# Stan994265/mVIL-Fusion

Hardware: AMD Instinct MI355X
Metric: sliding-window solve iterations/sec (10 KF, 1k feat, 30k LiDAR pts) (higher is better)
Workload: dtype f64; 1 GPU; BASELINE.json configs[1]: K=10 keyframes, L=1000 landmarks, 3068 visual factors, 24000 plane + 6000 edge LiDAR points, 9 IMU, 3 ICP, 4 LPS, prior n=70 (vil_marginalize of the preceding synthetic window, on the GPU); termination=function_tolerance, parallelism=1 GPU, step=one full window solve, inputs resident in HBM

## Files before the change

mvil-fusion_amd/csrc/vil_step.hpp:

```cpp
#pragma once
#include <type_traits>

#include "vil_dev.hpp"
#include "vil_factors.hpp"
#include "vil_finish.hpp"

namespace vd {

#define STEP_NB 4
#define CH_SLOTS 7
#define PF_N ((55 * 256 + VIL_STEP_THREADS - 1) / VIL_STEP_THREADS)

struct StepShared {
    Ctl c;
    double red[64];
    unsigned char tI[256], tJ[256];
    double xs[320], dinv[320];
    double y[320];
    double sc[320], dcs[320], gr[320], gn[320];
    double gd[320];
    double rt[320];
    double x0[328];
    unsigned char cst[48];
    double hs[12];
    int need, was_first, ok, cok;
    int hdr_posted, hdr_pad_;
    int early, judged;
    int done_at_entry, pad0_;
    long long tacc[6];
};

template <bool CMAX = false>
__device__ __forceinline__ void bsum3(double& a, double& b, double& c, StepShared& s) {
    a = wave_total_l63(a); b = wave_total_l63(b);
    c = CMAX ? wave_max_l63(c) : wave_total_l63(c);
    __syncthreads();
    const int w = vil_tid() >> 6, nw = blockDim.x >> 6;
    if ((vil_tid() & 63) == 63) { s.red[w] = a; s.red[8 + w] = b; s.red[16 + w] = c; }
    __syncthreads();
    a = 0; b = 0; c = 0;
    for (int q = 0; q < nw; ++q) { a += s.red[q]; b += s.red[8 + q]; c = CMAX ? fmax(c, s.red[16 + q]) : c + s.red[16 + q]; }
}

__device__ __forceinline__ void bsum5(double& a, double& b, double& c, double& d, double& e, StepShared& s) {
    a = wave_total_l63(a); b = wave_total_l63(b); c = wave_max_l63(c); d = wave_total_l63(d); e = wave_total_l63(e);
    __syncthreads();
    const int w = vil_tid() >> 6, nw = blockDim.x >> 6;
    if ((vil_tid() & 63) == 63) { s.red[w] = a; s.red[8 + w] = b; s.red[16 + w] = c; s.red[24 + w] = d; s.red[32 + w] = e; }
    __syncthreads();
    a = 0; b = 0; c = 0; d = 0; e = 0;
    for (int q = 0; q < nw; ++q) { a += s.red[q]; b += s.red[8 + q]; c = fmax(c, s.red[16 + q]); d += s.red[24 + q]; e += s.red[32 + q]; }
}

__device__ __forceinline__ void bsum6(double* v, StepShared& s) {
#pragma unroll
    for (int e = 0; e < 6; ++e) v[e] = wave_total_l63(v[e]);
    __syncthreads();
    const int w = vil_tid() >> 6, nw = blockDim.x >> 6;
    if ((vil_tid() & 63) == 63) { for (int e = 0; e < 6; ++e) s.red[8 * e + w] = v[e]; }
    __syncthreads();
#pragma unroll
    for (int e = 0; e < 6; ++e) { double a = 0; for (int q = 0; q < nw; ++q) a += s.red[8 * e + q]; v[e] = a; }
}

__device__ __forceinline__ double bsum(double v, StepShared& s) {
    v = wave_total_l63(v);
    __syncthreads();
    if ((vil_tid() & 63) == 63) s.red[vil_tid() >> 6] = v;
    __syncthreads();
    double t = 0;
    const int nw = blockDim.x >> 6;
    for (int w = 0; w < nw; ++w) t += s.red[w];
    return t;
}
__device__ __forceinline__ double bmax(double v, StepShared& s) {
    v = wave_max_l63(v);
    __syncthreads();
    if ((vil_tid() & 63) == 63) s.red[vil_tid() >> 6] = v;
    __syncthreads();
    double t = 0;
    const int nw = blockDim.x >> 6;
    for (int w = 0; w < nw; ++w) t = fmax(t, s.red[w]);
    return t;
}

struct LmRows { double e[13], a[6], b[6], c[6]; double m1, m2; int fs, fe, ac, c0, c1, c2, stride = 3; };
template <bool AG = false>
__device__ __forceinline__ void lm_rows(const DevP& P, const SysBuf& sb, int l, LmRows& r) {
    r.fs = P.glm_start[l]; r.fe = P.glm_start[l + 1]; r.ac = P.glm_acol[l];
    if (r.fe == r.fs) return;
    const double* e = sb.eA + (size_t)l * 13;
#pragma unroll
    for (int k = 0; k < 13; ++k) r.e[k] = ldx<AG>(e + k);
    const int f = r.fs, f1 = min(f + 1, r.fe - 1), f2 = min(f + 2, r.fe - 1);
    r.c0 = P.gfcol[f]; r.c1 = P.gfcol[f1]; r.c2 = P.gfcol[f2];
    const double* e0 = sb.eO + (size_t)f * 6; const double* e1 = sb.eO + (size_t)f1 * 6; const double* e2 = sb.eO + (size_t)f2 * 6;
#pragma unroll
    for (int k = 0; k < 6; ++k) { r.a[k] = ldx<AG>(e0 + k); r.b[k] = ldx<AG>(e1 + k); r.c[k] = ldx<AG>(e2 + k); }
    r.m1 = (f + 1 < r.fe) ? 1.0 : 0.0; r.m2 = (f + 2 < r.fe) ? 1.0 : 0.0;
}
template <bool AG = false>
__device__ __forceinline__ void lm_rows_quad(const DevP& P, const SysBuf& sb, int l, int qd, LmRows& r, const int G = 4 ) {
    const int fs0 = P.glm_start[l], fe = P.glm_start[l + 1];
    r.ac = qd == 0 ? P.glm_acol[l] : 0; r.stride = 3 * G;
    r.fs = min(fs0 + 3 * qd, fe); r.fe = fe;
    if (fe == fs0) { r.fs = fe; return; }
    const double* e = sb.eA + (size_t)l * 13;
#pragma unroll
    for (int k = 0; k < 13; ++k) { const double v = ldx<AG>(e + k); r.e[k] = qd == 0 ? v : 0.0; }
    const int f = min(fs0 + 3 * qd, fe - 1), f1 = min(f + 1, fe - 1), f2 = min(f + 2, fe - 1);
    r.c0 = P.gfcol[f]; r.c1 = P.gfcol[f1]; r.c2 = P.gfcol[f2];
    const double* e0 = sb.eO + (size_t)f * 6; const double* e1 = sb.eO + (size_t)f1 * 6; const double* e2 = sb.eO + (size_t)f2 * 6;
    const bool m0 = fs0 + 3 * qd < fe;
#pragma unroll
    for (int k = 0; k < 6; ++k) { const double va = ldx<AG>(e0 + k); r.a[k] = m0 ? va : 0.0; r.b[k] = ldx<AG>(e1 + k); r.c[k] = ldx<AG>(e2 + k); }
    r.m1 = (fs0 + 3 * qd + 1 < fe) ? 1.0 : 0.0; r.m2 = (fs0 + 3 * qd + 2 < fe) ? 1.0 : 0.0;
}
__device__ __forceinline__ double quad_total(double v) { v = dpp_add<0xB1, 0xf>(v); return dpp_add<0x4E, 0xf>(v); }
__device__ __forceinline__ double pair_total(double v) { return dpp_add<0xB1, 0xf>(v); }
template <bool AG = false>
__device__ __forceinline__ double lm_dot_rows(const DevP& P, const SysBuf& sb, const LmRows& r, const double* vc) {
    if (r.fe == r.fs) return 0.0;
    const double* e = r.e;
    const double* va = vc + r.ac; const double* vx = vc + col_ex(P);
    double s0 = e[0] * va[0], s1 = e[1] * va[1], s2 = e[2] * va[2], s3 = e[3] * va[3];
    s0 += e[4] * va[4]; s1 += e[5] * va[5];
    s2 += e[6] * vx[0]; s3 += e[7] * vx[1]; s0 += e[8] * vx[2]; s1 += e[9] * vx[3]; s2 += e[10] * vx[4]; s3 += e[11] * vx[5];
    s0 += e[12] * vc[col_td(P)];
    {
        const double* v0 = vc + r.c0; const double* v1 = vc + r.c1; const double* v2 = vc + r.c2;
        const double* a = r.a; const double* b = r.b; const double* c = r.c;
        s0 += a[0] * v0[0]; s1 += a[1] * v0[1]; s2 += a[2] * v0[2]; s3 += a[3] * v0[3]; s0 += a[4] * v0[4]; s1 += a[5] * v0[5];
        s2 += r.m1 * (b[0] * v1[0] + b[1] * v1[1] + b[2] * v1[2]); s3 += r.m1 * (b[3] * v1[3] + b[4] * v1[4] + b[5] * v1[5]);
        s0 += r.m2 * (c[0] * v2[0] + c[1] * v2[1] + c[2] * v2[2]); s1 += r.m2 * (c[3] * v2[3] + c[4] * v2[4] + c[5] * v2[5]);
    }
    for (int f = r.fs + r.stride; f < r.fe; f += r.stride) {
        const int f1 = min(f + 1, r.fe - 1), f2 = min(f + 2, r.fe - 1);
        const int c0 = P.gfcol[f], c1 = P.gfcol[f1], c2 = P.gfcol[f2];
        const double* e0 = sb.eO + (size_t)f * 6; const double* e1 = sb.eO + (size_t)f1 * 6; const double* e2 = sb.eO + (size_t)f2 * 6;
        double a[6], b[6], c[6];
#pragma unroll
        for (int k = 0; k < 6; ++k) { a[k] = ldx<AG>(e0 + k); b[k] = ldx<AG>(e1 + k); c[k] = ldx<AG>(e2 + k); }
        const double* v0 = vc + c0; const double* v1 = vc + c1; const double* v2 = vc + c2;
        const double m1 = (f + 1 < r.fe) ? 1.0 : 0.0, m2 = (f + 2 < r.fe) ? 1.0 : 0.0;
        s0 += a[0] * v0[0]; s1 += a[1] * v0[1]; s2 += a[2] * v0[2]; s3 += a[3] * v0[3]; s0 += a[4] * v0[4]; s1 += a[5] * v0[5];
        s2 += m1 * (b[0] * v1[0] + b[1] * v1[1] + b[2] * v1[2]); s3 += m1 * (b[3] * v1[3] + b[4] * v1[4] + b[5] * v1[5]);
        s0 += m2 * (c[0] * v2[0] + c[1] * v2[1] + c[2] * v2[2]); s1 += m2 * (c[3] * v2[3] + c[4] * v2[4] + c[5] * v2[5]);
    }
    return (s0 + s1) + (s2 + s3);
}
template <bool AG = false>
__device__ __forceinline__ double lm_dot(const DevP& P, const SysBuf& sb, int l, const double* vc) {
    LmRows r; lm_rows<AG>(P, sb, l, r);
    return lm_dot_rows<AG>(P, sb, r, vc);
}

__device__ __forceinline__ double quad_form(const DevP& P, const SysBuf& sb, const double* vc, const double* vl, StepShared& s) {
    const int D = P.D, L = P.L, t = vil_tid(), NT = blockDim.x;
    double part = 0;
    for (int e = t; e < D * D; e += NT) { const int i = e / D, j = e - i * D; part += vc[i] * sb.S[e] * vc[j]; }
    for (int l = t; l < L; l += NT) {
        const double ip = sb.invp[l];
        if (ip == 0.0) continue;
        const double ev = lm_dot(P, sb, l, vc);
        part += ip * ev * ev + 2.0 * vl[l] * ev + sb.hll[l] * vl[l] * vl[l];
    }
    return bsum(part, s);
}

__device__ __forceinline__ void pose_plus(const double* in, const double* d, double* o) {
    for (int k = 0; k < 3; ++k) o[k] = in[k] + d[k];
    Q4 q = qmul(qload(in + 3), Q4{1.0, 0.5 * d[3], 0.5 * d[4], 0.5 * d[5]});
    const double n = 1.0 / sqrt(q.w * q.w + q.x * q.x + q.y * q.y + q.z * q.z);
    o[3] = q.x * n; o[4] = q.y * n; o[5] = q.z * n; o[6] = q.w * n;
}


__host__ __device__ constexpr int tri_row_c(int q) { int I = 0; while ((I + 1) * (I + 2) / 2 <= q) ++I; return I; }
__host__ __device__ constexpr int tri_col_c(int q) { return q - tri_row_c(q) * (tri_row_c(q) + 1) / 2; }
template <int N, class F> __device__ __forceinline__ void static_for(F&& f) {
    if constexpr (N > 0) { static_for<N - 1>(f); f(std::integral_constant<int, N - 1>{}); }
}
static_assert(VIL_STEP_THREADS == 512, "the tile <-> element mapping above assumes two tiles per 512-thread stride");

__device__ __forceinline__ int tri_off(int i) { return (i * (i + 1)) >> 1; }
}
#include "vil_chain.hpp"
#include "vil_prechain.hpp"
namespace vd {

#define TILE_RS 17
#define TILE_SZ (16 * TILE_RS)
__device__ __forceinline__ int tl_base(int I, int J) { return (tri_off(I) + J) * TILE_SZ; }
__device__ __forceinline__ int tl_idx(int i, int j) { return tl_base(i >> 4, j >> 4) + (i & 15) * TILE_RS + (j & 15); }
__device__ __forceinline__ int tl_phys(int e) { return (e >> 8) * TILE_SZ + ((e >> 4) & 15) * TILE_RS + (e & 15); }

struct NoPre { template <class C> __device__ __forceinline__ void operator()(C*, const int*) const {} };
template <bool REGRES, class PTR, class PRE = NoPre>
__device__ __forceinline__ bool chol_blocked(PTR A, int D, StepShared& s, double* Acol = nullptr, PRE pre = PRE()) {
    const int t = vil_tid(), NT = blockDim.x, wave = t >> 6, lane = t & 63, NW = NT >> 6;
    const int R = D + 1;
    const int T = (R + 15) >> 4;
    const int la = (lane & 15) * TILE_RS + (lane >> 4);
    const int lc = (lane >> 4) * TILE_RS + (lane & 15);
#ifdef VIL_STAMPS
    long long tacc[6] = {0, 0, 0, 0, 0, 0}, tprev = 0;
    #define CSTAMP(k) do { long long tt_; asm volatile("s_memtime %0\n s_waitcnt lgkmcnt(0)" : "=s"(tt_) :: "memory"); if (k >= 0) tacc[k < 0 ? 0 : k] += tt_ - tprev; tprev = tt_; } while (0)
#else
    #define CSTAMP(k) do {} while (0)
#endif
    const int ntile_all = (T * (T + 1)) >> 1;
    d4 Creg[REGRES ? CH_SLOTS : 1]; int tIJ[REGRES ? CH_SLOTS : 1];
    if constexpr (REGRES) {
#pragma unroll
        for (int u = 0; u < CH_SLOTS; ++u) {
            const int g = wave + NW * u;
            tIJ[u] = -1;
            if (g < ntile_all) {
                const int I = s.tI[g], J = s.tJ[g];
                tIJ[u] = (I << 8) | J;
                const int cb = tl_base(I, J) + lc;
#pragma unroll
                for (int q = 0; q < 4; ++q) Creg[u][q] = A[cb + q * (4 * TILE_RS)];
            }
        }
        pre(Creg, tIJ);
    }
    for (int kb = 0; kb < D; kb += STEP_NB) {
        const int nb = min(STEP_NB, D - kb);
        const int Kt = kb >> 4, ko = kb & 15;
        CSTAMP(-1);
        if constexpr (REGRES) if (ko == 0) {
#pragma unroll
            for (int u = 0; u < CH_SLOTS; ++u) if (tIJ[u] >= 0 && (tIJ[u] & 255) == Kt) {
                const int cb = tl_base(tIJ[u] >> 8, Kt) + lc;
#pragma unroll
                for (int q = 0; q < 4; ++q) A[cb + q * (4 * TILE_RS)] = Creg[u][q];
            }
            __syncthreads();
            CSTAMP(4);
        }
        if constexpr (!REGRES) if (ko == 0) {
            __syncthreads();
            for (int e = t; e < (T - Kt) * TILE_SZ; e += NT) { const int I = Kt + e / TILE_SZ, w = e - (I - Kt) * TILE_SZ; Acol[e] = A[tl_base(I, Kt) + w]; }
            __syncthreads();
        }
        double* const AC = REGRES ? (double*)A : Acol;
        auto cbase = [&](int I) { return REGRES ? tl_base(I, Kt) : (I - Kt) * TILE_SZ; };
        const int db = cbase(Kt) + ko * TILE_RS + ko;
        double d00 = AC[db], d10 = 0, d11 = 1, d20 = 0, d21 = 0, d22 = 1, d30 = 0, d31 = 0, d32 = 0, d33 = 1;
        if (nb > 1) { d10 = AC[db + TILE_RS]; d11 = AC[db + TILE_RS + 1]; }
        if (nb > 2) { d20 = AC[db + 2 * TILE_RS]; d21 = AC[db + 2 * TILE_RS + 1]; d22 = AC[db + 2 * TILE_RS + 2]; }
        if (nb > 3) { d30 = AC[db + 3 * TILE_RS]; d31 = AC[db + 3 * TILE_RS + 1]; d32 = AC[db + 3 * TILE_RS + 2]; d33 = AC[db + 3 * TILE_RS + 3]; }
        double l00, r0_, l11, r1_, l22, r2_, l33, r3_;
        bool ok = d00 > 0.0 && isfinite(d00);
        sqrt_rsqrt(d00, l00, r0_);
        const double l10 = d10 * r0_, l20 = d20 * r0_, l30 = d30 * r0_;
        d11 -= l10 * l10; ok = ok && d11 > 0.0 && isfinite(d11);
        sqrt_rsqrt(d11, l11, r1_);
        const double l21 = (d21 - l20 * l10) * r1_, l31 = (d31 - l30 * l10) * r1_;
        d22 -= l20 * l20 + l21 * l21; ok = ok && d22 > 0.0 && isfinite(d22);
        sqrt_rsqrt(d22, l22, r2_);
        const double l32 = (d32 - l30 * l20 - l31 * l21) * r2_;
        d33 -= l30 * l30 + l31 * l31 + l32 * l32; ok = ok && d33 > 0.0 && isfinite(d33);
        sqrt_rsqrt(d33, l33, r3_);
        if (!ok) return false;
        CSTAMP(0);
        const int r0 = kb + nb;
        for (int i = r0 + t; i < R; i += NT) {
            const int base = cbase(i >> 4) + (i & 15) * TILE_RS + ko;
            const double a0 = AC[base], a1 = nb > 1 ? AC[base + 1] : 0.0, a2 = nb > 2 ? AC[base + 2] : 0.0, a3 = nb > 3 ? AC[base + 3] : 0.0;
            const double x0 = a0 * r0_;
            const double x1 = (a1 - x0 * l10) * r1_;
            const double x2 = (a2 - x0 * l20 - x1 * l21) * r2_;
            const double x3 = (a3 - x0 * l30 - x1 * l31 - x2 * l32) * r3_;
            AC[base] = x0; if (nb > 1) AC[base + 1] = x1; if (nb > 2) AC[base + 2] = x2; if (nb > 3) AC[base + 3] = x3;
        }
        if (t == NT - 2) {
            AC[db] = l00; s.dinv[kb] = r0_;
            if (nb > 1) { AC[db + TILE_RS] = l10; AC[db + TILE_RS + 1] = l11; s.dinv[kb + 1] = r1_; }
            if (nb > 2) { AC[db + 2 * TILE_RS] = l20; AC[db + 2 * TILE_RS + 1] = l21; AC[db + 2 * TILE_RS + 2] = l22; s.dinv[kb + 2] = r2_; }
            if (nb > 3) { AC[db + 3 * TILE_RS] = l30; AC[db + 3 * TILE_RS + 1] = l31; AC[db + 3 * TILE_RS + 2] = l32; AC[db + 3 * TILE_RS + 3] = l33; s.dinv[kb + 3] = r3_; }
        }
        CSTAMP(5);
        __syncthreads();
        CSTAMP(1);
        const bool kk = (lane >> 4) < nb;
        if constexpr (REGRES) {
#pragma unroll
            for (int u = 0; u < CH_SLOTS; ++u) {
                const int I = tIJ[u] >> 8, J = tIJ[u] & 255;
                if (tIJ[u] < 0 || J < Kt) continue;
                if (J > Kt) {
                    const double a_ = A[tl_base(I, Kt) + la + ko], b_ = A[tl_base(J, Kt) + la + ko];
                    const double av = kk ? -a_ : 0.0, bv = kk ? b_ : 0.0;
                    Creg[u] = __builtin_amdgcn_mfma_f64_16x16x4f64(av, bv, Creg[u], 0, 0, 0);
                } else if (r0 < R) {
                    const int rr = (I << 4) + (lane & 15), cr = (J << 4) + (lane & 15);
                    const double a_ = A[tl_base(I, Kt) + la + ko], b_ = A[tl_base(J, Kt) + la + ko];
                    const double av = (rr >= r0 && rr < R && kk) ? a_ : 0.0;
                    const double bv = (cr >= r0 && cr < D && kk) ? b_ : 0.0;
                    d4 z = {0.0, 0.0, 0.0, 0.0};
                    const d4 acc = __builtin_amdgcn_mfma_f64_16x16x4f64(av, bv, z, 0, 0, 0);
                    const int cb = tl_base(I, J) + lc;
#pragma unroll
                    for (int g = 0; g < 4; ++g) A[cb + g * (4 * TILE_RS)] -= acc[g];
                }
            }
        } else { if (r0 < R) {
            {
                const int I0 = r0 >> 4, nact = T - I0;
                for (int u0 = wave; u0 < nact; u0 += NW) {
                    const int I = I0 + u0;
                    const int rr = (I << 4) + (lane & 15), cr = (Kt << 4) + (lane & 15);
                    const double a_ = AC[cbase(I) + la + ko], b_ = AC[cbase(Kt) + la + ko];
                    const double av = (rr >= r0 && rr < R && kk) ? a_ : 0.0, bv = (cr >= r0 && cr < D && kk) ? b_ : 0.0;
                    d4 z = {0.0, 0.0, 0.0, 0.0};
                    const d4 acc = __builtin_amdgcn_mfma_f64_16x16x4f64(av, bv, z, 0, 0, 0);
                    const int cb = cbase(I) + lc;
#pragma unroll
                    for (int g = 0; g < 4; ++g) AC[cb + g * (4 * TILE_RS)] -= acc[g];
                }
            }
            const bool col_done = (ko + nb >= 16) || (kb + nb >= D);
            if (col_done && Kt + 1 < T) {
                __syncthreads();
                const int I0 = Kt + 1, n = T - I0, ntile = n * (n + 1) / 2;
                const int kv = min(16, D - (Kt << 4));
                for (int t0 = 0; t0 < ntile; t0 += 4 * NW) {
                    d4 acc[4]; int cb[4];
                    const int cnt = min(4, (ntile - t0 - wave + NW - 1) / NW);
// ... 90 lines not shown
            for (int r = 0; r < 4; ++r)
#pragma unroll
                for (int q = 0; q < 4; ++q) xd[r][q] = (FULL || r < nb) ? A[pb + r * TILE_RS + q] : 0.0;
#pragma unroll
            for (int q = 0; q < 4; ++q) xr[q] = A[pr + q];
#pragma unroll
            for (int q = 0; q < 4; ++q) {
                d00 = fma(-xd[0][q], xd[0][q], d00);
                d10 = fma(-xd[1][q], xd[0][q], d10); d11 = fma(-xd[1][q], xd[1][q], d11);
                d20 = fma(-xd[2][q], xd[0][q], d20); d21 = fma(-xd[2][q], xd[1][q], d21); d22 = fma(-xd[2][q], xd[2][q], d22);
                d30 = fma(-xd[3][q], xd[0][q], d30); d31 = fma(-xd[3][q], xd[1][q], d31); d32 = fma(-xd[3][q], xd[2][q], d32); d33 = fma(-xd[3][q], xd[3][q], d33);
                a0 = fma(-xr[q], xd[0][q], a0); a1 = fma(-xr[q], xd[1][q], a1); a2 = fma(-xr[q], xd[2][q], a2); a3 = fma(-xr[q], xd[3][q], a3);
            }
        }
        double l00 = 0, r0_, l11 = 0, r1_, l22 = 0, r2_, l33 = 0, r3_;
        if constexpr (DIAG) rsqrt_sqrt(d00, l00, r0_); else r0_ = rsqrt_1(d00);
        const double l10 = d10 * r0_, l20 = d20 * r0_, l30 = d30 * r0_, x0 = a0 * r0_;
        d11 = fma(-l10, l10, d11);
        const double t21 = fma(-l20, l10, d21), t31 = fma(-l30, l10, d31), u22 = fma(-l20, l20, d22), u33a = fma(-l30, l30, d33), v32 = fma(-l30, l20, d32);
        const double y1 = fma(-x0, l10, a1), y2a = fma(-x0, l20, a2), y3a = fma(-x0, l30, a3);
        if constexpr (DIAG) rsqrt_sqrt(d11, l11, r1_); else r1_ = rsqrt_1(d11);
        const double l21 = t21 * r1_, l31 = t31 * r1_, x1 = y1 * r1_;
        d22 = fma(-l21, l21, u22);
        const double t32 = fma(-l31, l21, v32), u33 = fma(-l31, l31, u33a), y2 = fma(-x1, l21, y2a), y3b = fma(-x1, l31, y3a);
        if constexpr (DIAG) rsqrt_sqrt(d22, l22, r2_); else r2_ = rsqrt_1(d22);
        const double l32 = t32 * r2_, x2 = y2 * r2_;
        d33 = fma(-l32, l32, u33);
        const double y3 = fma(-x2, l32, y3b);
        if constexpr (DIAG) rsqrt_sqrt(d33, l33, r3_); else r3_ = rsqrt_1(d33);
        const double x3 = y3 * r3_;
        const bool ok = (r0_ + r1_) + (r2_ + r3_) < 1.7976931348623157e308;
        if constexpr (FULL) { const int pad = rowb + 16; A[row ? base : pad] = x0; A[row ? base + 1 : pad] = x1; A[row ? base + 2 : pad] = x2; A[row ? base + 3 : pad] = x3; }
        else if (row) { A[base] = x0; if (nb > 1) A[base + 1] = x1; if (nb > 2) A[base + 2] = x2; if (nb > 3) A[base + 3] = x3; }
        if (tp == 0) {
            if (!ok) s.cok = 0;
            s.dinv[kb] = r0_;
            if (nb > 1) { A[db + TILE_RS] = l10; s.dinv[kb + 1] = r1_; }
            if (nb > 2) { A[db + 2 * TILE_RS] = l20; A[db + 2 * TILE_RS + 1] = l21; s.dinv[kb + 2] = r2_; }
            if (nb > 3) { A[db + 3 * TILE_RS] = l30; A[db + 3 * TILE_RS + 1] = l31; A[db + 3 * TILE_RS + 2] = l32; s.dinv[kb + 3] = r3_; }
            if constexpr (DIAG) { A[db] = l00; if (nb > 1) A[db + TILE_RS + 1] = l11; if (nb > 2) A[db + 2 * TILE_RS + 2] = l22; if (nb > 3) A[db + 3 * TILE_RS + 3] = l33; }
        }
    };
#pragma unroll
    for (int u = 0; u < SLOTS; ++u) if (tIJ[u] >= 0 && (tIJ[u] & 255) == 0) {
        const int cb = tl_base(tIJ[u] >> 8, 0) + lc;
#pragma unroll
        for (int q = 0; q < 4; ++q) A[cb + q * (4 * TILE_RS)] = Creg[u][q];
    }
    lds_barrier();
    if (tp >= 0) { if (D >= STEP_NB) diag_panel(0, std::true_type{}, std::false_type{}); else diag_panel(0, std::false_type{}, std::false_type{}); }
    lds_barrier();
    if (!s.cok) return false;
    for (int kb = 0; kb + STEP_NB < D; kb += STEP_NB) {
        const int Kt = kb >> 4, ko = kb & 15;
        const int kb1 = kb + STEP_NB, Kn = kb1 >> 4;
        const int c0 = kb1 + min(STEP_NB, D - kb1);
        if (tp >= 0) { if (kb1 + STEP_NB <= D) diag_panel(kb1, std::true_type{}, std::true_type{}); else diag_panel(kb1, std::false_type{}, std::true_type{}); }
        const int Kc = c0 >> 4, cs = c0 & 15;
#pragma unroll
        for (int u = 0; u < SLOTS; ++u) {
            const int I = tIJ[u] >> 8, J = tIJ[u] & 255;
            if (tIJ[u] < 0 || J < Kc) continue;
            const double a_ = A[tl_base(I, Kt) + la + ko], b_ = A[tl_base(J, Kt) + la + ko];
            Creg[u] = __builtin_amdgcn_mfma_f64_16x16x4f64(-a_, b_, Creg[u], 0, 0, 0);
            if (J == Kc && c0 < D) {
                const int cl = lane & 15;
                if (cl >= cs && cl < cs + STEP_NB) {
                    const int cb = tl_base(I, J) + lc;
#pragma unroll
                    for (int q = 0; q < 4; ++q) A[cb + q * (4 * TILE_RS)] = Creg[u][q];
                }
            }
        }
        lds_barrier();
    }
    return s.cok != 0;
}

__device__ __forceinline__ double bcast_lane(const double v, const int src) {
    return __hiloint2double(__builtin_amdgcn_readlane(__double2hiint(v), src), __builtin_amdgcn_readlane(__double2loint(v), src));
}
template <bool FIRST, bool FULL, int NTC = 0, class PTR>
__device__ __forceinline__ bool rowwave_panel(PTR A, const int Kt, const int D, const int R, StepShared& s, const int lane) {
    constexpr int o = FIRST ? 4 : 0;
    const int c0 = Kt << 4;
    const int nt = FULL ? 16 : NTC > 0 ? NTC : min(16, D - c0);
    const int row = c0 + o + lane, rc = min(row, R - 1);
    const int base = tl_base(rc >> 4, Kt) + (rc & 15) * TILE_RS;
    double t[16];
#pragma unroll
    for (int c = 0; c < 16; ++c) t[c] = A[base + c];
    double l10 = 0, l20 = 0, l21 = 0, l30 = 0, l31 = 0, l32 = 0, r4_[4] = {0, 0, 0, 0};
    if constexpr (FIRST) {
        const double d00 = A[0], d10 = A[TILE_RS], d20 = A[2 * TILE_RS], d21 = A[2 * TILE_RS + 1], d30 = A[3 * TILE_RS], d31 = A[3 * TILE_RS + 1], d32 = A[3 * TILE_RS + 2];
        double d11 = A[TILE_RS + 1], d22 = A[2 * TILE_RS + 2], d33 = A[3 * TILE_RS + 3];
        r4_[0] = rsqrt_1(d00);
        l10 = d10 * r4_[0]; l20 = d20 * r4_[0]; l30 = d30 * r4_[0];
        d11 = fma(-l10, l10, d11);
        const double t21 = fma(-l20, l10, d21), t31 = fma(-l30, l10, d31), u22 = fma(-l20, l20, d22), u33a = fma(-l30, l30, d33), v32 = fma(-l30, l20, d32);
        r4_[1] = rsqrt_1(d11);
        l21 = t21 * r4_[1]; l31 = t31 * r4_[1];
        d22 = fma(-l21, l21, u22);
        const double t32 = fma(-l31, l21, v32), u33 = fma(-l31, l31, u33a);
        r4_[2] = rsqrt_1(d22);
        l32 = t32 * r4_[2];
        d33 = fma(-l32, l32, u33);
        r4_[3] = rsqrt_1(d33);
        if (lane == 0) { A[TILE_RS] = l10; A[2 * TILE_RS] = l20; A[2 * TILE_RS + 1] = l21; A[3 * TILE_RS] = l30; A[3 * TILE_RS + 1] = l31; A[3 * TILE_RS + 2] = l32; }
    }
    auto B = [&](const int c, const int m) -> double {
        if constexpr (FIRST) { if (c < 4) return c == 1 ? l10 : c == 2 ? (m == 0 ? l20 : l21) : (m == 0 ? l30 : m == 1 ? l31 : l32); }
        return bcast_lane(t[m], c - o);
    };
    double rlast = 0.0;
#pragma unroll
    for (int k = 0; k < 16; ++k) {
        if (FULL || k < nt) {
            double r;
            if (FIRST && k < 4) {
                if (k >= 1) t[k] = fma(-t[k - 1], B(k, k - 1), t[k]);
                r = r4_[k];
            } else {
                if (k >= 1) t[k] = fma(-t[k - 1], B(k, k - 1), t[k]);
                r = rsqrt_1(bcast_lane(t[k], k - o));
            }
            t[k] *= r;
            s.dinv[c0 + k] = r;
            rlast = r;
#pragma unroll
            for (int c = k + 2; c < 16; ++c) if (FULL || c < nt) t[c] = fma(-t[k], B(c, k), t[c]);
        }
    }
    if (row < R) {
#pragma unroll
        for (int c = 0; c < 16; ++c) if (FULL || c < nt) A[base + c] = t[c];
    }
    return rlast < 1.7976931348623157e308;
}
template <bool FIRST, bool PROG , class PTR>
__device__ __forceinline__ bool rowwave_panel_full(PTR A, const int Kt, const int R, StepShared& s, const int lane) {
    constexpr int o = FIRST ? 4 : 0;
    const int c0 = Kt << 4;
    const int rc = min(c0 + o + lane, R - 1);
    const int base = tl_base(rc >> 4, Kt) + (rc & 15) * TILE_RS;
    const int db = tl_base(Kt, Kt);
    double t[16];
#pragma unroll
    for (int c = 0; c < 16; ++c) t[c] = A[base + c];
    double l10 = 0, l20 = 0, l21 = 0, l30 = 0, l31 = 0, l32 = 0, r4_[4] = {0, 0, 0, 0};
    if constexpr (FIRST) {
        const double d00 = A[0], d10 = A[TILE_RS], d20 = A[2 * TILE_RS], d21 = A[2 * TILE_RS + 1], d30 = A[3 * TILE_RS], d31 = A[3 * TILE_RS + 1], d32 = A[3 * TILE_RS + 2];
        double d11 = A[TILE_RS + 1], d22 = A[2 * TILE_RS + 2], d33 = A[3 * TILE_RS + 3];
        r4_[0] = rsqrt_1(d00);
        l10 = d10 * r4_[0]; l20 = d20 * r4_[0]; l30 = d30 * r4_[0];
        d11 = fma(-l10, l10, d11);
        const double t21 = fma(-l20, l10, d21), t31 = fma(-l30, l10, d31), u22 = fma(-l20, l20, d22), u33a = fma(-l30, l30, d33), v32 = fma(-l30, l20, d32);
        r4_[1] = rsqrt_1(d11);
        l21 = t21 * r4_[1]; l31 = t31 * r4_[1];
        d22 = fma(-l21, l21, u22);
        const double t32 = fma(-l31, l21, v32), u33 = fma(-l31, l31, u33a);
        r4_[2] = rsqrt_1(d22);
        l32 = t32 * r4_[2];
        d33 = fma(-l32, l32, u33);
        r4_[3] = rsqrt_1(d33);
        if (lane == 0) { A[TILE_RS] = l10; A[2 * TILE_RS] = l20; A[2 * TILE_RS + 1] = l21; A[3 * TILE_RS] = l30; A[3 * TILE_RS + 1] = l31; A[3 * TILE_RS + 2] = l32; }
    }
    auto L4 = [&](const int c, const int m) -> double { return c == 1 ? l10 : c == 2 ? (m == 0 ? l20 : l21) : (m == 0 ? l30 : m == 1 ? l31 : l32); };
    auto Bfast = [&](const int c, const int m) -> double {
        if constexpr (FIRST) { if (c < 4) return L4(c, m); }
        return bcast_lane(t[m], c - o);
    };
    double bv[16], bn[16];
    double r = 0.0;
#pragma unroll
    for (int k = 0; k < 16; ++k) {
        if (k >= 1 && k + 2 < 16) {
#pragma unroll
            for (int c = k + 2; c < 16; ++c) { if (FIRST && c < 4) bn[c] = L4(c, k - 1); else bn[c] = A[db + c * TILE_RS + (k - 1)]; }
        }
        __builtin_amdgcn_sched_barrier(0);
        if (k >= 2) {
#pragma unroll
            for (int c = k + 1; c < 16; ++c) t[c] = fma(-t[k - 2], bv[c], t[c]);
        }
        if (k >= 1 && k + 1 < 16) t[k + 1] = fma(-t[k - 1], Bfast(k + 1, k - 1), t[k + 1]);
        if (k >= 1) t[k] = fma(-t[k - 1], Bfast(k, k - 1), t[k]);
        r = (FIRST && k < 4) ? r4_[k] : rsqrt_1(bcast_lane(t[k], k - o));
        t[k] *= r;
        s.dinv[c0 + k] = r;
        A[base + k] = t[k];
        if constexpr (PROG) { asm volatile("" ::: "memory"); __hip_atomic_store(&s.pad0_, (Kt << 5) + k + 1, __ATOMIC_RELAXED, __HIP_MEMORY_SCOPE_WORKGROUP); }
        __builtin_amdgcn_sched_barrier(0);
#pragma unroll
        for (int c = 0; c < 16; ++c) bv[c] = bn[c];
    }
    return r < 1.7976931348623157e308;
}
template <class PTR>
__device__ __forceinline__ void rowwave_panel_second(PTR A, const int Kt, const int o, const int R, StepShared& s, const int lane) {
    const int c0 = Kt << 4;
    const int rc = min(c0 + o + 64 + lane, R - 1);
    const int base = tl_base(rc >> 4, Kt) + (rc & 15) * TILE_RS;
    const int db = tl_base(Kt, Kt);
    double t[16];
#pragma unroll
    for (int c = 0; c < 16; ++c) t[c] = A[base + c];
#pragma unroll
    for (int k = 0; k < 16; ++k) {
        double b[16], r;
        for (;;) {
            const int pv = __hip_atomic_load(&s.pad0_, __ATOMIC_RELAXED, __HIP_MEMORY_SCOPE_WORKGROUP);
            asm volatile("" ::: "memory");
#pragma unroll
            for (int m = 0; m < k; ++m) b[m] = A[db + k * TILE_RS + m];
            r = s.dinv[c0 + k];
            asm volatile("" ::: "memory");
            if (__builtin_amdgcn_readfirstlane(pv) >= (Kt << 5) + k + 1) break;
            __builtin_amdgcn_s_sleep(1);
        }
#pragma unroll
        for (int m = 0; m < k; ++m) t[k] = fma(-t[m], b[m], t[k]);
        t[k] *= r;
        A[base + k] = t[k];
    }
}
template <int SLOTS = 3, class PTR, class PRE = NoPre>
__device__ __forceinline__ bool chol_rowwave(PTR A, int D, StepShared& s, PRE pre = PRE()) {
    const int t = vil_tid(), NT = blockDim.x, wave = t >> 6, lane = t & 63, NW = NT >> 6;
    const int R = D + 1, T = (R + 15) >> 4, TD = (D + 15) >> 4;
    const int la = (lane & 15) * TILE_RS + (lane >> 4);
    const int lc = (lane >> 4) * TILE_RS + (lane & 15);
    const int ntile_all = (T * (T + 1)) >> 1;
    const int npw = R - 4 > 64 ? 2 : 1;
    const int NWP = NW - npw;
    const int n_idle = (ntile_all <= (NWP - npw) * SLOTS && NWP >= 4) ? npw : 0;
    const int NWT = NWP - n_idle;
    const bool idle_w = wave < NWP && wave >= NWP - 4 && wave < NWP - 4 + n_idle;
    const int wr = wave - (wave >= NWP - 4 + n_idle && wave < NWP ? n_idle : 0);
    d4 Creg[SLOTS]; int tIJ[SLOTS];
#pragma unroll
    for (int u = 0; u < SLOTS; ++u) {
        const int g = idle_w ? ntile_all : (wave < NWP ? wr + NWT * u : NWT * SLOTS + (wave - NWP) + npw * u);
        tIJ[u] = -1;
        if (g < ntile_all) {
            const int I = s.tI[g], J = s.tJ[g];
            tIJ[u] = (I << 8) | J;
            const int cb = tl_base(I, J) + lc;
#pragma unroll
            for (int q = 0; q < 4; ++q) Creg[u][q] = A[cb + q * (4 * TILE_RS)];
        }
    }
    pre(Creg, tIJ);
    if (t == 0) { s.cok = 1; s.pad0_ = 0; }
#pragma unroll
    for (int u = 0; u < SLOTS; ++u) if (tIJ[u] >= 0 && (tIJ[u] & 255) == 0) {
        const int cb = tl_base(tIJ[u] >> 8, 0) + lc;
#pragma unroll
        for (int q = 0; q < 4; ++q) A[cb + q * (4 * TILE_RS)] = Creg[u][q];
    }
    lds_barrier();
    auto update = [&](const int u, const int Kt) {
        const int I = tIJ[u] >> 8, J = tIJ[u] & 255;
        const int ab = tl_base(I, Kt) + la, bb = tl_base(J, Kt) + la;
        double a_[4], b_[4];
#pragma unroll
        for (int q = 0; q < 4; ++q) { a_[q] = A[ab + 4 * q]; b_[q] = A[bb + 4 * q]; }
        d4 c0 = __builtin_amdgcn_mfma_f64_16x16x4f64(-a_[0], b_[0], Creg[u], 0, 0, 0), c1 = __builtin_amdgcn_mfma_f64_16x16x4f64(-a_[1], b_[1], d4{0.0, 0.0, 0.0, 0.0}, 0, 0, 0);
        c0 = __builtin_amdgcn_mfma_f64_16x16x4f64(-a_[2], b_[2], c0, 0, 0, 0); c1 = __builtin_amdgcn_mfma_f64_16x16x4f64(-a_[3], b_[3], c1, 0, 0, 0);
#pragma unroll
        for (int q = 0; q < 4; ++q) Creg[u][q] = c0[q] + c1[q];
    };
    for (int Kt = 0; Kt < TD; ++Kt) {
        const int o = Kt == 0 ? 4 : 0;
        const bool two = R - (Kt << 4) - o > 64;
        if (wave == NWP) {
            bool ok;
            if (two) ok = Kt == 0 ? rowwave_panel_full<true, true>(A, 0, R, s, lane) : rowwave_panel_full<false, true>(A, Kt, R, s, lane);
            else ok = Kt == 0 ? rowwave_panel_full<true, false>(A, 0, R, s, lane) : (D - (Kt << 4) >= 16 ? rowwave_panel_full<false, false>(A, Kt, R, s, lane) : D - (Kt << 4) == 3 ? rowwave_panel<false, false, 3>(A, Kt, D, R, s, lane) : D - (Kt << 4) == 15 ? rowwave_panel<false, false, 15>(A, Kt, D, R, s, lane) : rowwave_panel<false, false>(A, Kt, D, R, s, lane));
            if (!ok && lane == 0) s.cok = 0;
        } else if (two && wave == NWP + 1) rowwave_panel_second(A, Kt, o, R, s, lane);
        lds_barrier();
        if (Kt + 1 >= TD) break;
#pragma unroll
        for (int u = 0; u < SLOTS; ++u) if (tIJ[u] >= 0 && (tIJ[u] & 255) == Kt + 1) {
            update(u, Kt);
            const int cb = tl_base(tIJ[u] >> 8, Kt + 1) + lc;
#pragma unroll
            for (int q = 0; q < 4; ++q) A[cb + q * (4 * TILE_RS)] = Creg[u][q];
        }
        lds_barrier();
#pragma unroll
        for (int u = 0; u < SLOTS; ++u) if (tIJ[u] >= 0 && (tIJ[u] & 255) > Kt + 1) update(u, Kt);
    }
    return s.cok != 0;
}
template <int SLOTS, class PTR, class PRE = NoPre>
__device__ __forceinline__ bool chol_dense(PTR A, int D, StepShared& s, PRE pre = PRE()) {
    if (D >= 16 && D + 1 <= 132 && (blockDim.x >> 6) >= 8) return chol_rowwave<SLOTS>(A, D, s, pre);
    return chol_lookahead<SLOTS, false>(A, D, s, pre);
}

template <class PTR>
__device__ __forceinline__ void back_subst_cols(PTR A, int D, StepShared& s) {
    const int t = vil_tid(), NT = blockDim.x, wave = t >> 6, lane = t & 63;
    const int TD = (D + 15) >> 4;
    for (int i = t; i < (TD << 4); i += NT) { s.y[i] = i < D ? A[tl_idx(D, i)] : 0.0; s.xs[i] = 0.0; }
    const int g = lane >> 4, j = lane & 15;
    auto prepare = [&](const int blk, double* l, double& sc) {
        const int nb = min(16, D - (blk << 4)), cb = blk - g, ccb = max(cb, 0), col = (ccb << 4) + j;
        const bool valid = cb >= 0;
        const int tb = tl_base(blk, ccb) + j;
#pragma unroll
        for (int i = 0; i < 16; ++i) l[i] = A[tb + i * TILE_RS];
        sc = g == 0 ? s.dinv[min(col, D - 1)] : 1.0;
#pragma unroll
        for (int i = 0; i < 16; ++i) { double v = l[i]; asm volatile("" : "+v"(v)); l[i] = (valid && i < nb && (g > 0 || i > j)) ? v * sc : 0.0; }
    };
    __syncthreads();
    for (int blk = TD - 1; blk >= 0; --blk) {
        const int nb = min(16, D - (blk << 4));
        if (wave == 0) {
            const int cb = blk - g, col = (max(cb, 0) << 4) + j;
            double l[16], sc;
            prepare(blk, l, sc);
            double yv = s.y[col];
            if (g == 0) yv = (yv - s.xs[col]) * sc;
            if (nb == 16) {
#pragma unroll
                for (int i = 15; i >= 0; --i) yv = fma(-l[i], bcast_lane(yv, i), yv);
            } else {
#pragma unroll
                for (int i = 15; i >= 0; --i) if (i < nb) yv = fma(-l[i], bcast_lane(yv, i), yv);
            }
            if (cb >= 0) s.y[col] = yv;
        }
        __syncthreads();
        if (wave > 0 && blk >= 4) {
            for (int c = t - 64; c < ((blk - 3) << 4); c += NT - 64) {
                const int cb = tl_base(blk, c >> 4) + (c & 15);
                double acc = 0.0;
                for (int i = 0; i < nb; ++i) acc = fma(A[cb + i * TILE_RS], s.y[(blk << 4) + i], acc);
                s.xs[c] += acc;
            }
        }
    }
}

template <class PTR>
__device__ __forceinline__ void back_subst(PTR A, int D, StepShared& s) {
    const int t = vil_tid(), NT = blockDim.x, wave = t >> 6, lane = t & 63;
    for (int i = t; i < D; i += NT) s.y[i] = A[tl_idx(D, i)];
    const int TD = (D + 15) >> 4;
    for (int i = D + t; i < (TD << 4); i += NT) s.y[i] = 0.0;
    {
        const int j = lane >> 2, p = lane & 3;
        const int lc = (lane >> 4) * TILE_RS + (lane & 15);
        for (int tt = wave; tt < TD; tt += NT >> 6) {
            const int n_t = min(16, D - (tt << 4));
            const int tb = tl_base(tt, tt);
            const double* dv = s.dinv + (tt << 4);
            double dr[16], lq[16][4], wq[4] = {0.0, 0.0, 0.0, 0.0};
#pragma unroll
            for (int i = 0; i < 16; ++i) dr[i] = dv[i];
#pragma unroll
            for (int i = 1; i < 16; ++i)
#pragma unroll
                for (int m = 0; m < (i + 3) / 4; ++m) lq[i][m] = A[tb + i * TILE_RS + 4 * m + p];
#pragma unroll
            for (int i = 1; i < 16; ++i)
#pragma unroll
                for (int m = 0; m < (i + 3) / 4; ++m) { double v = lq[i][m]; asm volatile("" : "+v"(v)); lq[i][m] = (4 * m + p < i) ? v : 0.0; }
            const bool col = j < n_t;
#pragma unroll
            for (int i = 0; i < 16; ++i) {
                double a0 = 0.0, a1 = 0.0;
#pragma unroll
                for (int m = 0; m < (i + 3) / 4; ++m) { if (m & 1) a1 = fma(lq[i][m], wq[m], a1); else a0 = fma(lq[i][m], wq[m], a0); }
                double sum = a0 + a1;
                if (i > 0) { sum = dpp_add<0xB1, 0xf>(sum); sum = dpp_add<0x4E, 0xf>(sum); }
                double off = -sum * dr[i], on = dr[i];
                asm volatile("" : "+v"(off), "+v"(on));
                const bool live = col && i < n_t;
                const double wi = (live && i > j) ? off : ((live && i == j) ? on : 0.0);
                wq[i >> 2] = ((i & 3) == p) ? wi : wq[i >> 2];
            }
#pragma unroll
            for (int m = 0; m < 4; ++m) A[tb + j * TILE_RS + 4 * m + p] = wq[m];
            if (tt > 0) {
                const int nb = tl_base(tt, tt - 1);
                asm volatile("s_waitcnt lgkmcnt(0)" ::: "memory");
                double av[4], bv[4];
#pragma unroll
                for (int q = 0; q < 4; ++q) { const int o = (4 * q + (lane >> 4)) * TILE_RS + (lane & 15); av[q] = A[tb + o]; bv[q] = A[nb + o]; }
                d4 c = {0.0, 0.0, 0.0, 0.0};
#pragma unroll
                for (int q = 0; q < 4; ++q) {
                    double b_ = bv[q]; asm volatile("" : "+v"(b_));
                    c = __builtin_amdgcn_mfma_f64_16x16x4f64(av[q], (4 * q + (lane >> 4) < n_t) ? b_ : 0.0, c, 0, 0, 0);
                }
#pragma unroll
                for (int g = 0; g < 4; ++g) A[nb + lc + g * (4 * TILE_RS)] = c[g];
            }
        }
    }
    lds_barrier();
#ifdef VIL_STAMPS
    if (t == 0) { long long tt_; asm volatile("s_memtime %0\n s_waitcnt lgkmcnt(0)" : "=s"(tt_) :: "memory"); s.tacc[0] = tt_; }
#endif
    double crit = 0.0;
    for (int blk = TD - 1; blk >= 0; --blk) {
        const int kb = blk << 4;
        if (t < 64) {
            const int tt = t & 15;
            const int tb = tl_base(blk, blk) + tt * TILE_RS;
            const int nb = tl_base(blk, max(blk - 1, 0)) + tt;
            double wr[16], nn[16];
#pragma unroll
            for (int i = 0; i < 16; ++i) { wr[i] = A[tb + i]; nn[i] = A[nb + i * TILE_RS]; }
            const double yo = s.y[kb + tt] - crit;
            s.y[kb + tt] = yo;
            asm volatile("s_waitcnt lgkmcnt(0)" ::: "memory");
            double a0 = 0.0, a1 = 0.0, a2 = 0.0, a3 = 0.0, c0 = 0.0, c1 = 0.0, c2 = 0.0, c3 = 0.0;
#pragma unroll
            for (int i = 0; i < 16; i += 4) {
                const double y0 = s.y[kb + i], y1 = s.y[kb + i + 1], y2 = s.y[kb + i + 2], y3 = s.y[kb + i + 3];
                a0 = fma(wr[i], y0, a0); a1 = fma(wr[i + 1], y1, a1); a2 = fma(wr[i + 2], y2, a2); a3 = fma(wr[i + 3], y3, a3);
                c0 = fma(nn[i], y0, c0); c1 = fma(nn[i + 1], y1, c1); c2 = fma(nn[i + 2], y2, c2); c3 = fma(nn[i + 3], y3, c3);
            }
            asm volatile("s_waitcnt lgkmcnt(0)" ::: "memory");
            s.y[kb + tt] = (a0 + a1) + (a2 + a3);
            crit = (c0 + c1) + (c2 + c3);
        }
        lds_barrier();
        if (t >= 64) {
            const int lim = kb - 16;
            for (int w0 = (t & ~63) - 64; w0 < lim; w0 += NT - 64) {
                const int c = w0 + (t & 63), cc = min(c, lim - 1);
                const int base = tl_base(blk, cc >> 4) + (cc & 15);
                double v0 = 0.0, v1 = 0.0, v2 = 0.0, v3 = 0.0;
#pragma unroll
                for (int r = 0; r < 16; r += 4) {
                    v0 = fma(A[base + r * TILE_RS], s.y[kb + r], v0);
                    v1 = fma(A[base + (r + 1) * TILE_RS], s.y[kb + r + 1], v1);
                    v2 = fma(A[base + (r + 2) * TILE_RS], s.y[kb + r + 2], v2);
                    v3 = fma(A[base + (r + 3) * TILE_RS], s.y[kb + r + 3], v3);
                }
                double yn = s.y[cc] - ((v0 + v1) + (v2 + v3));
                asm volatile("" : "+v"(yn));
                if (c < lim) s.y[cc] = yn;
            }
        }
    }
    lds_barrier();
}

struct ChainSrcStep {
    const double* S; int D; const double* sc_; const double* dcs_; const double* gd_; const double* u_; double mu;
    __device__ __forceinline__ double u(int i) const { return u_[i]; }
    int NP;
    __device__ __forceinline__ double raw(int i, int j) const { return S[(size_t)i * D + j]; }
    __device__ __forceinline__ double diag(int k, int i, int j) const { return raw(NP + 9 * k + i, NP + 9 * k + j); }
    __device__ __forceinline__ double sub(int k, int kn, int q, int c) const { return raw(NP + 9 * kn + q, NP + 9 * k + c); }
    __device__ __forceinline__ double prow(int r, int k, int c) const { return raw(r, NP + 9 * k + c); }
    __device__ __forceinline__ double sc(int j) const { return sc_[j]; }
    __device__ __forceinline__ double madd(int j) const { const double d = dcs_[j]; return mu * d * d; }
    __device__ __forceinline__ double rowscale(int r) const { return sc_[r]; }
    __device__ __forceinline__ double rhsraw(int j) const { return gd_[j]; }
    __device__ __forceinline__ void row_done(int, int r, double zr, double& q) const { q += 2.0 * u_[r] * zr; }
    __device__ __forceinline__ void wput(double* p, double v) const { *p = v; }
};

template <bool WLDS, class PUB, class SIDE>
__device__ __forceinline__ bool solve_chain(const DevP& P, const SysBuf& sb, StepShared& s, double* lds, const double mu, const bool cam, double& qpart, PUB pub, SIDE side) {
    const int t = vil_tid();
#ifdef VIL_STAMPS
    #define SSTAMP(k) do { if (t == 0) { long long tt_; asm volatile("s_memtime %0\n s_waitcnt lgkmcnt(0)" : "=s"(tt_) :: "memory"); P.dbg[40 + k] = tt_; } } while (0)
#else
    #define SSTAMP(k) do {} while (0)
#endif
    SSTAMP(0);
    const int K = P.K, D = P.D, NP = P.NV, R = NP + 1, T = (R + 15) >> 4, ntile = (T * (T + 1)) >> 1;
    const int RS = P.chain_rs, NB = 9 * K, m = K >> 1;
    double* Tl = lds;
    double* Wt = WLDS ? lds + ntile * TILE_SZ : P.M;
    const ChainLds L = chain_lds(lds + ntile * TILE_SZ + (WLDS ? (size_t)chain_wcols(K) * RS : 0), K);
    if (t < 8) chain_flag_set(L.flag + t, 0);
    __syncthreads();
    SSTAMP(1);
    if (t < 384) {
        const ChainSrcStep src{sb.S, D, s.sc, s.dcs, s.gd, s.y, mu, NP};
        double qc = 0.0;
        if (cam) chain_eliminate<true>(src, K, NP, RS, Wt, L, qc, P.dbg); else chain_eliminate<false>(src, K, NP, RS, Wt, L, qc, P.dbg);
        qpart += qc;
    } else {
        const int pl = t - 384, NE = ntile << 8;
        for (int e0 = pl; e0 < NE; e0 += 4 * 128) {
            double v[4]; int ii[4], jj[4];
#pragma unroll
            for (int u = 0; u < 4; ++u) {
                const int e = min(e0 + 128 * u, NE - 1), tile = e >> 8, w = e & 255;
                ii[u] = (s.tI[tile] << 4) + (w >> 4); jj[u] = (s.tJ[tile] << 4) + (w & 15);
                v[u] = sb.S[(size_t)min(ii[u], NP - 1) * D + min(jj[u], NP - 1)];
            }
#pragma unroll
            for (int u = 0; u < 4; ++u) {
                const int e = e0 + 128 * u;
                if (e >= NE) break;
                const int i = ii[u], j = jj[u];
                double mv = 0.0;
                if (i < NP && j <= i) {
                    if (cam) qpart += (i == j ? 1.0 : 2.0) * s.y[i] * v[u] * s.y[j];
                    mv = s.sc[i] * v[u] * s.sc[j];
                    if (i == j) mv += mu * s.dcs[i] * s.dcs[i];
                } else if (i == NP && j < NP) mv = s.sc[j] * s.gd[j];
                Tl[tl_phys(e)] = mv;
            }
        }
#ifdef VIL_STAMPS
        if (t == 384) { long long tt_; asm volatile("s_memtime %0\n s_waitcnt lgkmcnt(0)" : "=s"(tt_) :: "memory"); P.dbg[57] = tt_; P.dbg[58] = tt_; }
#endif
    }
    __syncthreads();
    SSTAMP(2);
    if (chain_flag_get(L.flag + 5)) return false;
    SSTAMP(3);
    auto schur = [&](d4* Creg, const int* tIJ) {
        const int lane = t & 63, row = lane & 15, kq = lane >> 4;
        if (P.skip_mask & 128) return;
        const int RS4 = 4 * RS;
#pragma unroll
        for (int u = 0; u < CH_SLOTS; ++u) {
            if (tIJ[u] < 0) continue;
            const int I = tIJ[u] >> 8, J = tIJ[u] & 255;
            const bool va = (I << 4) + row < R, vb = (J << 4) + row < R;
            const double* pa = Wt + kq * RS + (I << 4) + row;
            const double* pb = Wt + kq * RS + (J << 4) + row;
            d4 c4 = Creg[u];
            for (int kk = 0; kk < NB; kk += 32) {
                const double* qa = pa + kk * RS; const double* qb = pb + kk * RS;
                double av[8], bv[8];
#pragma unroll
                for (int g = 0; g < 8; ++g) { av[g] = qa[g * RS4]; bv[g] = qb[g * RS4]; }
#pragma unroll
                for (int g = 0; g < 8; ++g) {
                    const bool kv = kk + 4 * g + kq < NB;
                    c4 = __builtin_amdgcn_mfma_f64_16x16x4f64((va && kv) ? -av[g] : 0.0, (vb && kv) ? bv[g] : 0.0, c4, 0, 0, 0);
                }
            }
            Creg[u] = c4;
        }
    };
    if (!chol_lookahead<CH_SLOTS, false>(Tl, NP, s, schur)) return false;
    SSTAMP(4);
    back_subst(Tl, NP, s);
    pub();
    SSTAMP(5);
    double* tB = L.tB;
    {
        const int G = (4 * NB <= VIL_STEP_THREADS) ? 4 : 2;
        const int j = t / G, part = t - j * G;
        const int jc = min(j, NB - 1);
        double acc = 0.0;
        for (int rr = part; rr < NP; rr += G) acc += Wt[(size_t)jc * RS + rr] * s.y[rr];
        acc += __shfl_xor(acc, 1, 64);
        if (G == 4) acc += __shfl_xor(acc, 2, 64);
        if (j < NB && part == 0) tB[j] = Wt[(size_t)j * RS + NP] - acc;
    }
    __syncthreads();
    if (t < 64) chain_block_back(L.Ldg + 54 * m, nullptr, tB + 9 * m, nullptr, s.y + NP + 9 * m);
    __syncthreads();
    if (t < 64) { for (int k = m - 1; k >= 0; --k) chain_block_back(L.Ldg + 54 * k, L.Lsb + 82 * k, tB + 9 * k, s.y + NP + 9 * (k + 1), s.y + NP + 9 * k); }
    else if (t < 128) { for (int k = m + 1; k < K; ++k) chain_block_back(L.Ldg + 54 * k, L.Lsb + 82 * k, tB + 9 * k, s.y + NP + 9 * (k - 1), s.y + NP + 9 * k); }
    else if (t >= VIL_STEP_THREADS - 64) side();
    __syncthreads();
    SSTAMP(6);
    return true;
}

template <bool RW , class PUB, class SIDE>
__device__ __forceinline__ bool solve_prechain(const DevP& P, const SysBuf& sb, StepShared& s, double* lds, const double mu, const bool cam, double& qpart, const int epoch , PUB pub, SIDE side) {
    const int t = vil_tid();
    SSTAMP(0);
    const int K = P.K, D = P.D, NP = P.NV, R = NP + 1, T = (R + 15) >> 4, ntile = (T * (T + 1)) >> 1;
    const int RS = P.chain_rs, NB = 9 * K, m = K >> 1;
    double* Tl = lds;
    const double* Wt = P.chW;
    double* Ldg = lds + ntile * TILE_SZ; double* Lsb = Ldg + 54 * K; double* tB = Lsb + 82 * K;
    {
        const int NE = ntile << 8;
        for (int e0 = t; e0 < NE; e0 += 8 * VIL_STEP_THREADS) {
            double v[8]; int ii[8], jj[8];
#pragma unroll
            for (int u = 0; u < 8; ++u) {
                const int e = min(e0 + VIL_STEP_THREADS * u, NE - 1), tile = e >> 8, w = e & 255;
                ii[u] = (s.tI[tile] << 4) + (w >> 4); jj[u] = (s.tJ[tile] << 4) + (w & 15);
                v[u] = ld_ag(sb.S + (size_t)min(ii[u], NP - 1) * D + min(jj[u], NP - 1));
            }
#pragma unroll
            for (int u = 0; u < 8; ++u) {
                const int e = e0 + VIL_STEP_THREADS * u;
                if (e >= NE) break;
                const int i = ii[u], j = jj[u];
                double mv = 0.0;
                if (i < NP && j <= i) {
                    if (cam) qpart += (i == j ? 1.0 : 2.0) * s.y[i] * v[u] * s.y[j];
                    mv = s.sc[i] * v[u] * s.sc[j];
                    if (i == j) mv += mu * s.dcs[i] * s.dcs[i];
                } else if (i == NP && j < NP) mv = s.sc[j] * s.gd[j];
                Tl[tl_phys(e)] = mv;
            }
        }
    }
    if (P.rs_merged) {
        for (int i = t; i < P.n_ww; i += VIL_STEP_THREADS) spin_until_eq(P.wwflag + i, epoch, P.abortf);
        __syncthreads();
    }
    if (t == 0) prof_stamp(P, epoch - 1, 9);
    SSTAMP(1);
    const int f2 = (P.rs_merged || P.prechain == 2) ? ld_ag(P.chflag + 2) : 0;
    {
        const int NE = ntile << 8;
        for (int e0 = t; e0 < NE; e0 += 8 * VIL_STEP_THREADS) {
            double ww[8];
#pragma unroll
            for (int u = 0; u < 8; ++u) ww[u] = ld_ag(P.chWW + tl_phys(min(e0 + VIL_STEP_THREADS * u, NE - 1)));
#pragma unroll
            for (int u = 0; u < 8; ++u) {
                const int e = e0 + VIL_STEP_THREADS * u;
                if (e >= NE) break;
                const int tile = e >> 8, w = e & 255, i = (s.tI[tile] << 4) + (w >> 4), j = (s.tJ[tile] << 4) + (w & 15);
                if (i <= NP && j <= i && j < NP) Tl[tl_phys(e)] -= (i < NP ? s.sc[i] : 1.0) * ww[u] * s.sc[j];
            }
        }
        if (cam) {
            if (t < NP) qpart += 2.0 * s.y[t] * (ld_ag(P.chZ + t) + ld_ag(P.chZ + R + t));
            if (t == 0) qpart += ld_ag(P.chQ) + ld_ag(P.chQ + 1);
        }
        if (t == 0 && !ld_ag(P.chOk)) s.ok = 0;
    }
    __syncthreads();
    SSTAMP(2); SSTAMP(3);
    if (!s.ok) return false;
    const int G = (4 * NB <= VIL_STEP_THREADS) ? 4 : 2;
    const int j = t / G, part = t - j * G;
    const int jc = min(j, NB - 1);
    double wv[24], wrhs = 0.0;
    const bool small = ntile <= 24;
    if (small) {
// ... 779 lines not shown
```

Measured before the change: 17700 iterations/s.

## Pipeline block back-substitution across waves with LDS flag handoff instead of barriers

```diff
diff --git a/mvil-fusion_amd/csrc/vil_step.hpp b/mvil-fusion_amd/csrc/vil_step.hpp
--- a/mvil-fusion_amd/csrc/vil_step.hpp
+++ b/mvil-fusion_amd/csrc/vil_step.hpp
@@ -24,9 +24,11 @@
     unsigned char cst[48];
     double hs[12];
     int need, was_first, ok, cok;
-    int hdr_posted, hdr_pad_;
+    int hdr_posted;
+    int bs_fold;
     int early, judged;
-    int done_at_entry, pad0_;
+    int done_at_entry;
+    int pad0_;
     long long tacc[6];
 };
 
@@ -723,11 +725,19 @@
 
 template <class PTR>
 __device__ __forceinline__ void back_subst_cols(PTR A, int D, StepShared& s) {
-    const int t = vil_tid(), NT = blockDim.x, wave = t >> 6, lane = t & 63;
+    const int t = vil_tid(), NT = blockDim.x, wave = t >> 6, lane = t & 63, NW = NT >> 6;
     const int TD = (D + 15) >> 4;
+#ifdef VIL_BS_STAMPS
+    #define BSTAMP(k) do { if (lane == 0 && (k) < 41) { long long tt_; asm volatile("s_memtime %0\n s_waitcnt lgkmcnt(0)" : "=s"(tt_) :: "memory"); reinterpret_cast<long long*>(s.red)[k] = tt_; } } while (0)
+#else
+    #define BSTAMP(k) do {} while (0)
+#endif
+    if (wave == 0) BSTAMP(0);
     for (int i = t; i < (TD << 4); i += NT) { s.y[i] = i < D ? A[tl_idx(D, i)] : 0.0; s.xs[i] = 0.0; }
+    if (t == 0) { s.pad0_ = 0; s.bs_fold = 0; }
     const int g = lane >> 4, j = lane & 15;
-    auto prepare = [&](const int blk, double* l, double& sc) {
+    double l[16], sc = 1.0;
+    auto prepare = [&](const int blk) {
         const int nb = min(16, D - (blk << 4)), cb = blk - g, ccb = max(cb, 0), col = (ccb << 4) + j;
         const bool valid = cb >= 0;
         const int tb = tl_base(blk, ccb) + j;
@@ -737,34 +747,62 @@
 #pragma unroll
         for (int i = 0; i < 16; ++i) { double v = l[i]; asm volatile("" : "+v"(v)); l[i] = (valid && i < nb && (g > 0 || i > j)) ? v * sc : 0.0; }
     };
-    __syncthreads();
-    for (int blk = TD - 1; blk >= 0; --blk) {
-        const int nb = min(16, D - (blk << 4));
-        if (wave == 0) {
-            const int cb = blk - g, col = (max(cb, 0) << 4) + j;
-            double l[16], sc;
-            prepare(blk, l, sc);
-            double yv = s.y[col];
-            if (g == 0) yv = (yv - s.xs[col]) * sc;
-            if (nb == 16) {
-#pragma unroll
-                for (int i = 15; i >= 0; --i) yv = fma(-l[i], bcast_lane(yv, i), yv);
-            } else {
-#pragma unroll
-                for (int i = 15; i >= 0; --i) if (i < nb) yv = fma(-l[i], bcast_lane(yv, i), yv);
-            }
-            if (cb >= 0) s.y[col] = yv;
-        }
-        __syncthreads();
-        if (wave > 0 && blk >= 4) {
-            for (int c = t - 64; c < ((blk - 3) << 4); c += NT - 64) {
-                const int cb = tl_base(blk, c >> 4) + (c & 15);
+    auto recur = [&](double yv, const int nb, auto NBC) -> double {
+        constexpr int NB = decltype(NBC)::value;
+#pragma unroll
+        for (int i = 15; i >= 0; --i) if (NB ? i < NB : i < nb) yv = fma(-l[i], bcast_lane(yv, i), yv);
+        return yv;
+    };
+    auto turn = [&](const int blk) {
+        const int nb = min(16, D - (blk << 4)), cb = blk - g, col = (max(cb, 0) << 4) + j;
+        const int need = TD - 1 - blk, needf = max(TD - 4 - blk, 0);
+        double yv, xv;
+        for (;;) {
+            const int pv = __hip_atomic_load(&s.pad0_, __ATOMIC_RELAXED, __HIP_MEMORY_SCOPE_WORKGROUP), fv = __hip_atomic_load(&s.bs_fold, __ATOMIC_RELAXED, __HIP_MEMORY_SCOPE_WORKGROUP);
+            asm volatile("" ::: "memory");
+            yv = s.y[col]; xv = s.xs[col];
+            asm volatile("" ::: "memory");
+            const int ps = __builtin_amdgcn_readfirstlane(pv);
+            if (ps >= need && __builtin_amdgcn_readfirstlane(fv) >= needf) break;
+            if (ps + 2 < need) __builtin_amdgcn_s_sleep(8); else if (ps + 1 < need) __builtin_amdgcn_s_sleep(2); else __builtin_amdgcn_s_sleep(1);
+        }
+        BSTAMP(1 + 3 * blk);
+        if (g == 0) yv = (yv - xv) * sc;
+        if (nb == 16) yv = recur(yv, 16, std::integral_constant<int, 16>{}); else if (nb == 3) yv = recur(yv, 3, std::integral_constant<int, 3>{});
+        else if (nb == 15) yv = recur(yv, 15, std::integral_constant<int, 15>{}); else yv = recur(yv, nb, std::integral_constant<int, 0>{});
+        BSTAMP(2 + 3 * blk);
+        if (cb >= 0) s.y[col] = yv;
+        asm volatile("" ::: "memory");
+        __hip_atomic_store(&s.pad0_, blk ? TD - blk : 0, __ATOMIC_RELAXED, __HIP_MEMORY_SCOPE_WORKGROUP);
+        BSTAMP(3 + 3 * blk);
+        if (blk >= 4) {
+            const int nc = (blk - 3) << 4;
+            bool mine = false;
+            for (int c0 = 0; c0 < nc; c0 += 64) {
+                const int c = c0 + lane, cc = min(c, nc - 1);
+                const int ab = tl_base(blk, cc >> 4) + (cc & 15);
                 double acc = 0.0;
-                for (int i = 0; i < nb; ++i) acc = fma(A[cb + i * TILE_RS], s.y[(blk << 4) + i], acc);
-                s.xs[c] += acc;
-            }
-        }
-    }
+                for (int i = 0; i < nb; ++i) acc = fma(A[ab + i * TILE_RS], s.y[(blk << 4) + i], acc);
+                while (!mine) {
+                    const int fv = __hip_atomic_load(&s.bs_fold, __ATOMIC_RELAXED, __HIP_MEMORY_SCOPE_WORKGROUP);
+                    asm volatile("" ::: "memory");
+                    if (__builtin_amdgcn_readfirstlane(fv) >= need) mine = true; else __builtin_amdgcn_s_sleep(1);
+                }
+                if (c < nc) s.xs[c] += acc;
+            }
+            asm volatile("" ::: "memory");
+            __hip_atomic_store(&s.bs_fold, TD - blk, __ATOMIC_RELAXED, __HIP_MEMORY_SCOPE_WORKGROUP);
+        }
+    };
+    for (int blk = TD - 1 - wave, first = 1;; blk -= NW, first = 0) {
+        if (blk >= 0) prepare(blk);
+        if (first) lds_barrier();
+        if (blk < 0) break;
+        turn(blk);
+    }
+    lds_barrier();
+    if (wave == 0) BSTAMP(40);
+    #undef BSTAMP
 }
 
 template <class PTR>
```

After: 18000 iterations/s (median of 3 runs). +1.7%, better.
